# robotics-upo/social_force_window_planner

Hardware: AMD Instinct MI355X
Metric: scored trajectories/sec (v x w samples x steps) @ N pedestrians; cmd_vel match (higher is better)
Workload: dtype f64

## Files before the change

### social_force_window_planner_amd/csrc/sfw_kernels.hip

```cpp

#include "sfw_device.h"
#include "sfw_math.h"

#include <type_traits>

#include <math.h>
#include <stdlib.h>
#include <cmath>

namespace {

constexpr int WAVE = 64;

#pragma clang fp contract(off)

__device__ __forceinline__ unsigned cell_index(double a, double res, double inv_res) {
  const double q = a * inv_res;
  const double m = __builtin_trunc(q);
  const double d = q - m;
  if (d < 1e-9 || d > 1.0 - 1e-9) return static_cast<unsigned>(a / res);
  return static_cast<unsigned>(m);
}

__device__ __forceinline__ bool world_to_map(const sfw_launch &L, double inv_res, double wx, double wy, unsigned &mx,
// ... 563 lines not shown
template <bool BATCH> __device__ __forceinline__ late_launch late_args_of(late_launch rec) {
  if constexpr (!BATCH) {
    (void)rec;
    return late_args();
  } else {
    const __attribute__((address_space(4))) void *p = rec;
    asm volatile("" : "+s"(p));
    return static_cast<late_launch>(p);
  }
}

__device__ __forceinline__ void clock_probe(int which) {
  if (blockIdx.x != gridDim.x / 2 || threadIdx.x != 0) return;
  unsigned long long *const p = late_args()->clock_probe;
  if (!p) return;
  p[2 * which] = __builtin_readcyclecounter();
  p[2 * which + 1] = wall_clock64();
}

template <typename R> struct sfm_consts {
  sfwm::poly_consts pc;
  R lambda, neg_l2e_inv_gamma, l2_f_social, c_vel, c_ang;
};
struct agent_consts {
  double f_desired, inv_tau, dt, rr, inv_O, l2_f_obstacle, l2e_inv_sigma;
  double f_gaze, f_coherence, f_repulsion;
  const double *obstacles;
  int O, robot_id, obs_tasks;
};
__device__ __forceinline__ agent_consts load_agent_consts(late_launch La, bool f32) {
  agent_consts c;
  c.f_desired = La->k.f_desired;
  c.inv_tau = La->k.inv_tau;
  c.dt = La->dt;
  c.rr = La->k.rr;
  c.inv_O = La->k.inv_O;
  c.l2_f_obstacle = f32 ? static_cast<double>(La->k.f.l2_f_obstacle) : La->k.d.l2_f_obstacle;
  c.l2e_inv_sigma = f32 ? static_cast<double>(La->k.f.l2e_inv_sigma) : La->k.d.l2e_inv_sigma;
  c.f_gaze = La->p.sfm_force_factor_group_gaze;
  c.f_coherence = La->p.sfm_force_factor_group_coherence;
  c.f_repulsion = La->p.sfm_force_factor_group_repulsion;
  c.O = La->O;
  c.obstacles = La->obstacles;
  c.obs_tasks = La->k.obs_tasks;
  c.robot_id = La->agent_c[0].id;
  return c;
}

__device__ __forceinline__ double copysign_from(double mag, double sgn) { return __builtin_copysign(mag, sgn); }
__device__ __forceinline__ float copysign_from(float mag, double sgn) {
  return __builtin_copysignf(mag, static_cast<float>(sgn));
}

template <typename R, bool NORM_ONLY = false>
__device__ __forceinline__ void pair_force(const sfm_consts<R> &k, R dx, R dy, R wx, R wy, double cw, R &fx,
                                           R &fy) {
  using namespace sfwm;
  const R tiny = tiny_of<R>::v;
  R rd, dn, rl, il;
  const R d2 = fma(dx, dx, fma(dy, dy, tiny));
  rsqrt_sqrt(d2, rd, dn);
  const R ux = dx * rd, uy = dy * rd;
  const R ix = fma(k.lambda, wx, ux), iy = fma(k.lambda, wy, uy);
  const R l2 = fma(ix, ix, fma(iy, iy, tiny));
  rsqrt_sqrt(l2, rl, il);
  const R sn = fma(ix, uy, -(iy * ux));
  const R ncs = fma(-ix, ux, -(iy * uy));
  const R theta = angle_abs(k.pc, fabs(sn), ncs, rl, il);
  const R a = fmax(fma(dn * rl, k.neg_l2e_inv_gamma, k.l2_f_social), R(-1100));
  const R t2 = l2 * (theta * theta);
  R ev, ea;
#if SFW_SIGN_OF_ZERO
  exp2_fast2(k.pc, fma(k.c_vel, t2, a), fma(k.c_ang, t2, a), ev, ea);
#else
  exp2_fast2_gated(k.pc, fma(k.c_vel, t2, a), fma(k.c_ang, t2, a), cw, ev, ea);
#endif
  if constexpr (NORM_ONLY) {
    const R q = fma(ev, ev, ea * ea);
    R rq, nq;
    rsqrt_sqrt(fma(R(1), q, tiny), rq, nq);
    fx = q * rq;
    fy = R(0);
    return;
  }
  ea = copysign_from(ea, cw);
  const R gx = ix * rl, gy = iy * rl;
  fx = fma(ea, gy, -(ev * gx));
  fy = fma(-ev, gy, -(ea * gx));
}
template <typename R, bool NORM_ONLY = false>
__device__ __forceinline__ void pair_force_state(const sfm_consts<R> &k, double pix, double piy, double vix,
                                                 double viy, double pjx, double pjy, double vjx, double vjy,
                                                 R &fx, R &fy) {
  const double dx = pjx - pix, dy = pjy - piy, wx = vix - vjx, wy = viy - vjy;
  const double cw = fma(wx, dy, -(wy * dx));
  pair_force<R, NORM_ONLY>(k, R(dx), R(dy), R(wx), R(wy), cw, fx, fy);
}

__device__ __forceinline__ double fast_norm(double x, double y) {
  const double q = fma(x, x, y * y);
  double rs, sq;
  sfwm::rsqrt_sqrt(fmax(q, 1e-300), rs, sq);
  return q * rs;
}

__device__ __forceinline__ void desired_force(const agent_consts &k, double px, double py, double vx, double vy,
                                              bool has_goal, double gx, double gy, double gr, double dv, double &fx,
                                              double &fy) {
  const double ex = gx - px, ey = gy - py;
  double inv, en;
  sfwm::rsqrt_sqrt(fmax(fma(ex, ex, ey * ey), 1e-300), inv, en);
  if (has_goal && en > gr) {
    fx = k.f_desired * (ex * inv * dv - vx) * k.inv_tau;
    fy = k.f_desired * (ey * inv * dv - vy) * k.inv_tau;
  } else {
    fx = -vx * k.inv_tau;
    fy = -vy * k.inv_tau;
  }
}

constexpr int OBS_SEG = 16;
constexpr int OBS_AGENT_LANES = WAVE / OBS_SEG;
#ifndef SFW_OBS_KA
#define SFW_OBS_KA 4
#endif
constexpr int OBS_AGENTS_PER_LANE = SFW_OBS_KA;
typedef const __attribute__((address_space(4))) double *obs_global_ptr;
__device__ __forceinline__ obs_global_ptr obs_global(const double *obstacles) {
  return (obs_global_ptr)(const __attribute__((address_space(1))) double *)obstacles;
}
__device__ __forceinline__ double2 obs_point(const double2 *obs, int o) { return obs[o]; }
__device__ __forceinline__ double2 obs_point(obs_global_ptr obs, int o) { return double2{obs[2 * o], obs[2 * o + 1]}; }
#ifndef SFW_FLAT_PIPELINED
#define SFW_FLAT_PIPELINED false
#endif
#ifndef SFW_OBS_UNIFORM
#define SFW_OBS_UNIFORM 1
#endif
#ifndef SFW_OBS_UNIFORM_LDS
#define SFW_OBS_UNIFORM_LDS 1
#endif
#ifndef SFW_SKIP_EMPTY_K2
#define SFW_SKIP_EMPTY_K2 1
#endif
#ifndef SFW_OBS_UNROLL_SCALAR
#define SFW_OBS_UNROLL_SCALAR 4
#endif
template <typename R>
__device__ __forceinline__ void obstacle_term(const sfm_consts<R> &k, double2 q, double px, double py, R nis, R &ax, R &ay) {
// ... 162 lines not shown
    }
    if (seg_done) {
      tx += ax;
      ty += ay;
      ax = R(0);
      ay = R(0);
    }
  };
  auto advance = [&](int &o, int &e) {
    o += 4;
    if (o >= e) {
      o = e;
      e = min(e + L, O);
    }
    return o < O;
  };
  if (O > 0) {
    int o = 0, e = min(L, O);
    obs_group ga, gb;
    obs_group_issue(ga, obs);
    for (;;) {
      int o2 = o, e2 = e;
      const bool more = advance(o2, e2);
      obs_group_wait(ga);
      if (more) obs_group_issue(gb, obs + 2 * o2);
      eval(ga, min(4, e - o), o + 4 >= e);
      if (!more) break;
      o = o2;
      e = e2;
      const bool more2 = advance(o2, e2);
      obs_group_wait(gb);
      if (more2) obs_group_issue(ga, obs + 2 * o2);
      eval(gb, min(4, e - o), o + 4 >= e);
      if (!more2) break;
      o = o2;
      e = e2;
    }
  }
  tx_out = static_cast<double>(tx);
  ty_out = static_cast<double>(ty);
  scale = obstacle_scale<R>(k, c, radius);
}

__device__ __forceinline__ double swap_pair(double v) {
  const uint64_t u = __builtin_bit_cast(uint64_t, v);
  constexpr int QP_1032 = 0xB1;
  const uint32_t lo = static_cast<uint32_t>(__builtin_amdgcn_update_dpp(0, static_cast<int>(static_cast<uint32_t>(u)), QP_1032, 0xf, 0xf, true));
  const uint32_t hi = static_cast<uint32_t>(__builtin_amdgcn_update_dpp(0, static_cast<int>(static_cast<uint32_t>(u >> 32)), QP_1032, 0xf, 0xf, true));
  return __builtin_bit_cast(double, (static_cast<uint64_t>(hi) << 32) | lo);
}

struct lds_layout {
  double *px, *py, *vx, *vy, *fjx, *fjy, *fcx, *fcy;
  double2 *gcen;
  double2 *obs;
  sfw_robot_step *rsb;
  sfw_agent_const *ac;
  double *swp;
  double2 *opart;
  double *wr;
  double *oscale;
  int *hasgoal, *dead, *grp, *goff, *gmem;
  unsigned char *hasgoal8;
  int hg_stride;
  size_t bytes;
  static constexpr int REG_DEAD_CAP = 32;
  __host__ __device__ lds_layout(char *base, int A, int cap, int GA, int G, int O, int NG, int NM, bool consts,
                                 bool with_frc, bool obs_in_lds = false) {
    char *const base0 = base;
    auto take = [&](size_t n) {
      char *p = base;
      base += (n + 15) & ~size_t(15);
      return p;
    };
    const size_t plane = sizeof(double) * static_cast<size_t>(cap);
    px = reinterpret_cast<double *>(take(plane));
    py = reinterpret_cast<double *>(take(plane));
    vx = reinterpret_cast<double *>(take(plane));
    vy = reinterpret_cast<double *>(take(plane));
    fjx = reinterpret_cast<double *>(take(plane));
    fjy = reinterpret_cast<double *>(take(plane));
    if (with_frc) {
      fcx = reinterpret_cast<double *>(take(plane));
      fcy = reinterpret_cast<double *>(take(plane));
      rsb = reinterpret_cast<sfw_robot_step *>(take(sizeof(sfw_robot_step) * 2));
      swp = reinterpret_cast<double *>(take(sizeof(double) * GA));
      opart = reinterpret_cast<double2 *>(take(sizeof(double2) * (O > 0 ? (obs_in_lds ? 4 : 2) * 64 : 0)));
      wr = reinterpret_cast<double *>(take(sizeof(double) * (O > 0 ? 4 : 0)));
      oscale = reinterpret_cast<double *>(take(sizeof(double) * (O > 0 ? A : 0)));
      obs = reinterpret_cast<double2 *>(take(sizeof(double2) * (obs_in_lds ? O + 2 : 0)));
      if (!obs_in_lds) obs = nullptr;
      hasgoal8 = reinterpret_cast<unsigned char *>(take(static_cast<size_t>(GA)));
      hasgoal = nullptr;
      hg_stride = 1;
      dead = reinterpret_cast<int *>(take(sizeof(int) * G));
    } else {
      fcx = fcy = nullptr;
      opart = nullptr;
      wr = nullptr;
      oscale = nullptr;
      obs = nullptr;
      hasgoal = reinterpret_cast<int *>(take(plane));
      hasgoal8 = nullptr;
      hg_stride = 2;
      swp = reinterpret_cast<double *>(take(plane));
      dead = reinterpret_cast<int *>(take(sizeof(int) * REG_DEAD_CAP));
      rsb = reinterpret_cast<sfw_robot_step *>(take(sizeof(sfw_robot_step) * G));
    }
    ac = reinterpret_cast<sfw_agent_const *>(take(sizeof(sfw_agent_const) * (consts ? A : 0)));
    gcen = reinterpret_cast<double2 *>(take(sizeof(double2) * (NG > 0 ? G * NG : 0)));
    grp = reinterpret_cast<int *>(take(sizeof(int) * (NG > 0 ? A : 0)));
    goff = reinterpret_cast<int *>(take(sizeof(int) * (NG > 0 ? NG + 1 : 0)));
    gmem = reinterpret_cast<int *>(take(sizeof(int) * (NG > 0 && NM > 0 ? NM : 0)));
    bytes = static_cast<size_t>(base - base0);
  }
  __device__ __forceinline__ int hg(int sl) const { return hg_stride == 1 ? static_cast<int>(hasgoal8[sl]) : hasgoal[sl * hg_stride]; }
};
template <int CAP> struct reg_off {
  static constexpr int PY = 8 * CAP, VX = 16 * CAP, VY = 24 * CAP, FJX = 32 * CAP, FJY = 40 * CAP, HG = 48 * CAP, SW = 56 * CAP,
                       DEAD = 64 * CAP, RSB = 64 * CAP + 4 * lds_layout::REG_DEAD_CAP;
};

struct agent_k {
  double gx, gy, gr, dv, rad;
  int id;
};
__device__ __forceinline__ agent_k agent_k_of(const sfw_agent_const &c) {
  return agent_k{c.goal_x, c.goal_y, c.goal_radius, c.desired_velocity, c.radius, c.id};
}
__device__ __forceinline__ agent_k agent_k_lds(const lds_layout &s, int i) { return agent_k_of(s.ac[i]); }
__device__ __forceinline__ agent_k agent_k_global(const sfw_agent_const *agent_c, int i) { return agent_k_of(agent_c[i]); }

template <typename R>
__device__ double2 group_force(const sfm_consts<R> &k, const agent_consts &c, const lds_layout &s, int NG, int g, int A,
                               int i, int sl, double px, double py) {
  const sfw_agent_const ci = s.ac[i];
  const int q = s.grp[i];
  if (q < 0) return double2{0.0, 0.0};
  const int m0 = s.goff[q], m1 = s.goff[q + 1];
  if (m1 - m0 < 2) return double2{0.0, 0.0};
  const double n = static_cast<double>(m1 - m0), inv_n = sfwm::rcp_nr(n);
  const double2 csum = s.gcen[g * NG + q];
  const double cx = csum.x * inv_n, cy = csum.y * inv_n;
  const double ex = ci.goal_x - px, ey = ci.goal_y - py;
  double inv_en, en;
  sfwm::rsqrt_sqrt(fmax(fma(ex, ex, ey * ey), 1e-300), inv_en, en);
  const bool has_dir = s.hg(sl) && en > ci.goal_radius;
  const double ddx = has_dir ? ex * inv_en : 0.0, ddy = has_dir ? ey * inv_en : 0.0;
  double fx = 0.0, fy = 0.0;
  {
// ... 504 lines not shown
    if constexpr (GROUPS) add_group_forces(k, c);
      }

  const late_launch Le = late_args();
  if (Le->phase == SFW_PHASE_PREFIX) {
    sfw_cls_agent *const out_state = Le->out_state;
    const int64_t A_late = Le->A;
#pragma unroll
    for (int r = 0; r < NS; ++r)
      if (ok_[r] && static_cast<int>(g4_[r] >> 2) < Gn) {
        const uint32_t io = io_[r];
        sfw_cls_agent c;
        c.px = lds_at<double>(smem, io); c.py = lds_at<double>(smem, io + PY);
        c.vx = lds_at<double>(smem, io + VX); c.vy = lds_at<double>(smem, io + VY);
        c.fx = fx[r]; c.fy = fy[r]; c.sw = sw[r];
        const int2 cell = lds_at<int2>(smem, io + off::HG);
        c.hasgoal = cell.x;
        c.pad = 0;
        out_state[(first_local + static_cast<int64_t>(g4_[r] >> 2)) * A_late + (cell.y >> 1)] = c;
      }
    if (lane < Gn) Le->out_dead[first_local + lane] = s.dead[lane];
    clock_probe(1);
    return;
  }
  double sw_acc = 0.0;
#pragma unroll
  for (int r = 0; r < NS; ++r) {
    if (G == 1) sw_acc += ok_[r] ? sw[r] : 0.0;
    else if (ok_[r]) lds_at<double>(smem, io_[r] + off::SW) = sw[r];
  }
  finish_wave(s, lane, G, Gn, first_local, sw_acc);
  clock_probe(1);
}
template <typename R, int NS, bool GROUPS>
__global__ void __launch_bounds__(WAVE, (NS == 1 && !GROUPS) ? 6 : 1) sfw_social_kernel(const sfw_launch L, const int G) {
  sfwm::fp_mode_for_omod();
  extern __shared__ __attribute__((aligned(16))) char smem[];
  social_reg_wave<R, NS, GROUPS>(L, G, smem, blockIdx.x, gridDim.x);
}

__global__ void __launch_bounds__(256) sfw_pair_table_kernel(uint16_t *tab, int A, int n_entries, int n_dummy) {
  const int u = blockIdx.x * blockDim.x + threadIdx.x;
  if (u >= n_entries) return;
  const int P = A * (A - 1) / 2;
  int i = A + (u >= P ? (u - P) % n_dummy : 0), j = i;
  if (u < P) {
    const int row = u / A;
    i = u - row * A;
    j = i + row + 1;
    j = (j >= A) ? j - A : j;
  }
  tab[u] = static_cast<uint16_t>(8 * i);
  tab[n_entries + u] = static_cast<uint16_t>(8 * j);
}

__device__ __forceinline__ void load_pair_entries(const uint16_t *ti, const uint16_t *tj, uint32_t lane_off, uint32_t &io,
                                                  uint32_t &jo) {
#ifdef SFW_DBG_C_LOADS
  io = ti[lane_off / 2];
  jo = tj[lane_off / 2];
  return;
#endif
  asm volatile("s_nop 4\n\tglobal_load_ushort %0, %2, %3\n\tglobal_load_ushort %1, %2, %4"
               : "=&v"(io), "=&v"(jo)
               : "v"(lane_off), "s"(ti), "s"(tj));
}
__device__ __forceinline__ void wait_pair_entries(uint32_t &io, uint32_t &jo) {
  asm volatile("s_waitcnt vmcnt(0)" : "+v"(io), "+v"(jo));
}

#ifndef SFW_FIRST_PAIRS_IN_REGS
#define SFW_FIRST_PAIRS_IN_REGS 1
#endif
#ifndef SFW_FLAT_WAVES
#define SFW_FLAT_WAVES 5
#endif
#ifndef SFW_FLAT_WAVES_NOOBS
#define SFW_FLAT_WAVES_NOOBS 6
#endif
__device__ __forceinline__ void wave_sync() {
  __builtin_amdgcn_fence(__ATOMIC_RELEASE, "wavefront");
  __builtin_amdgcn_wave_barrier();
  __builtin_amdgcn_fence(__ATOMIC_ACQUIRE, "wavefront");
}
struct cycle_result {
  double social_work;
  int dead;
  int ready;
  int fdone;
  int legal;
  double base0, base;
};
__device__ __forceinline__ int cycle_wait_ready(const cycle_result *res, int need) {
  int r;
  while ((r = *const_cast<const volatile int *>(&res->ready)) < need) __builtin_amdgcn_s_sleep(1);
  __builtin_amdgcn_fence(__ATOMIC_ACQUIRE, "workgroup");
  return r;
}
#define K2_SYNC() do { if constexpr (CYCLE) wave_sync(); else __syncthreads(); } while (0)
template <typename R, bool GROUPS, int CAP, bool OBS, bool CYCLE, bool BATCH = false>
__device__ __forceinline__ void social_flat_wave(const sfw_launch &L, char *const smem, const k1s_lds *const k1, cycle_result *const res,
                                                 const unsigned bid, const unsigned nblk, const int64_t item_base,
                                                 const late_launch Lb = nullptr) {
  static_assert(CYCLE || !BATCH, "a batched wave is a cycle kernel's wave");
  const int lane = threadIdx.x;
  const int A = L.A, O = L.O;
  const int NG = GROUPS ? L.NG : 0;
  const int cap = CAP > 0 ? CAP : ((A + 2) & ~1);
  const int PY = 8 * cap, VX = 16 * cap, VY = 24 * cap, FJX = 32 * cap, FJY = 40 * cap, FCX = 48 * cap,
            FCY = 56 * cap;
  (void)FCX;
  (void)FCY;
  constexpr bool CONSTS_IN_LDS = GROUPS || CYCLE;
  const lds_layout s(smem, A, cap, A, 1, O, NG, GROUPS ? L.n_grp_mem : 0, CONSTS_IN_LDS, true, L.k.obs_lds != 0);
  const int64_t first_local = CYCLE ? static_cast<int64_t>(bid) : item_base + xcd_contiguous(bid, nblk, static_cast<unsigned>(L.n_xcd));
  const sfm_consts<R> k0 = make_consts<R, true>(L);
  const sfw_force_k<R> &fk = force_k<R>(L);
  const R s_lambda = sfwm::sgpr_const(fk.lambda), s_nig = sfwm::sgpr_const(fk.neg_l2e_inv_gamma), s_lfs = sfwm::sgpr_const(fk.l2_f_social),
          s_cvel = sfwm::sgpr_const(fk.c_vel), s_cang = sfwm::sgpr_const(fk.c_ang);
  constexpr bool F32 = sizeof(R) == 4;
  const int step_begin = L.step_begin, step_end = L.step_end;
  if constexpr (CYCLE) {
    stage_consts<GROUPS, CONSTS_IN_LDS>(L, s, lane);
    if (lane == 0) s.dead[0] = 0;
    wave_sync();
  } else {
    if (!stage_wave<GROUPS, GROUPS>(L, s, lane, 1, 1, first_local)) {
      if (L.phase == SFW_PHASE_SUFFIX) finish_wave(s, lane, 1, 1, first_local, 0.0);
      if (L.phase == SFW_PHASE_PREFIX && lane == 0) L.out_dead[first_local] = s.dead[0];
      return;
    }
  }
  if constexpr (!BATCH) clock_probe(0);
  const int64_t rsample_v = CYCLE ? 0 : robot_sample_of_item(L, first_local);
  const int64_t rsample = static_cast<int64_t>(
      (static_cast<uint64_t>(static_cast<uint32_t>(__builtin_amdgcn_readfirstlane(static_cast<int>(rsample_v >> 32)))) << 32) |
      static_cast<uint32_t>(__builtin_amdgcn_readfirstlane(static_cast<int>(rsample_v))));

  if (!CYCLE && L.resume) {
    const sfw_cls_agent *rec = L.in_state + source_class_of_item(L, first_local) * A;
    for (int sl = lane; sl < A; sl += WAVE) {
      const sfw_cls_agent c = rec[sl];
      s.px[sl] = c.px;
      s.py[sl] = c.py;
      s.vx[sl] = c.vx;
      s.vy[sl] = c.vy;
      s.hasgoal8[sl] = static_cast<unsigned char>(c.hasgoal != 0);
      s.swp[sl] = c.sw;
      s.fcx[sl] = c.fx;
      s.fcy[sl] = c.fy;
      s.fjx[sl] = s.fjy[sl] = 0.0;
    }
  } else {
    const agent_consts c0 = load_agent_consts(late_args_of<BATCH>(Lb), F32);
    for (int sl = lane; sl < A; sl += WAVE) {
      const double px = L.agent_pos[2 * sl], py = L.agent_pos[2 * sl + 1];
      const double vx = L.agent_vel[2 * sl], vy = L.agent_vel[2 * sl + 1];
      const sfw_agent_const c = L.agent_c[sl];
      s.px[sl] = px;
      s.py[sl] = py;
      s.vx[sl] = vx;
      s.vy[sl] = vy;
      s.hasgoal8[sl] = static_cast<unsigned char>(c.has_goal != 0);
      s.swp[sl] = 0.0;
      double fx = 0.0, fy = 0.0;
// ... 29 lines not shown
    K2_SYNC();
    for (int sl = lane; sl < A; sl += WAVE)
      if (s.grp[sl] >= 0) {
        atomicAdd(&s.gcen[s.grp[sl]].x, s.px[sl]);
        atomicAdd(&s.gcen[s.grp[sl]].y, s.py[sl]);
      }
    K2_SYNC();
    for (int sl = lane; sl < A; sl += WAVE)
      if (sl != 0) {
        const double2 gf = group_force<R>(k, c, s, NG, 0, A, sl, sl, s.px[sl], s.py[sl]);
        s.fcx[sl] += gf.x;
        s.fcy[sl] += gf.y;
      }
    K2_SYNC();
  };
  if constexpr (GROUPS) {
    if (!L.resume) add_group_forces(k0, load_agent_consts(late_args_of<BATCH>(Lb), F32));
  }

  const int P = A * (A - 1) / 2;
  const int n_it = (P + WAVE - 1) / WAVE;
  const uint16_t *const tab_i = L.pair_tab, *const tab_j = L.pair_tab + static_cast<size_t>(n_it) * WAVE;
  const uint32_t lane_off = 2u * static_cast<uint32_t>(lane);

  const int64_t unit_vel_v = CYCLE ? 0 : L.rstep_stride + vel_row_of(L, rsample);
  const int64_t unit_pos = rsample,
                unit_vel = static_cast<int64_t>(
                    (static_cast<uint64_t>(static_cast<uint32_t>(__builtin_amdgcn_readfirstlane(static_cast<int>(unit_vel_v >> 32)))) << 32) |
                    static_cast<uint32_t>(__builtin_amdgcn_readfirstlane(static_cast<int>(unit_vel_v))));
  auto fetch_robot = [&](const sfw_unit *ptab, int64_t row_units, int st, int buf) {
    if constexpr (CYCLE) return;
    int l2 = lane;
    asm volatile("" : "+v"(l2));
    if (l2 < 2) {
      const char *src = reinterpret_cast<const char *>(ptab + static_cast<int64_t>(st) * row_units + (l2 ? unit_vel : unit_pos));
      __builtin_amdgcn_global_load_lds((const __attribute__((address_space(1))) void *)src,
                                       (__attribute__((address_space(3))) void *)(reinterpret_cast<char *>(s.rsb + buf)), 16,
                                       0, 0);
    }
  };
  if (step_begin < step_end) fetch_robot(L.ptab, L.row_units, step_begin, step_begin & 1);
  constexpr bool FIRST_IN_REGS = SFW_FIRST_PAIRS_IN_REGS && CAP == 64;
  uint32_t i0 = 0, j0 = 0;
  if constexpr (FIRST_IN_REGS) {
    if (n_it > 0) {
      load_pair_entries(tab_i, tab_j, lane_off, i0, j0);
      wait_pair_entries(i0, j0);
    }
  }

#if defined(SFW_ABL_HALF_LDS)
  double abl_ix = s.px[lane < A ? lane : 0], abl_iy = s.py[lane < A ? lane : 0], abl_fx = 0.0, abl_fy = 0.0;
#endif
  auto pair_at = [&](const sfm_consts<R> &k, uint32_t io, uint32_t jo) {
    R qx, qy;
    if constexpr (CAP > 0) {
      double pix, piy, vix, viy, pjx, pjy, vjx, vjy;
#if defined(SFW_ABL_NOREAD)
      pix = static_cast<double>(io); piy = 1.0; vix = 0.3; viy = 0.5; pjx = static_cast<double>(jo) * 0.37; pjy = -3.0; vjx = 0.25; vjy = static_cast<double>(jo) * 0.001;
#elif defined(SFW_ABL_HALF_LDS)
      pix = abl_ix; piy = abl_iy; vix = 0.3; viy = 0.5;
      asm volatile("ds_read_b64 %0, %4\n\tds_read_b64 %1, %4 offset:%5\n\tds_read_b64 %2, %4 offset:%6\n\tds_read_b64 %3, %4 offset:%7\n\ts_waitcnt lgkmcnt(0)"
                   : "=&v"(pjx), "=&v"(pjy), "=&v"(vjx), "=&v"(vjy) : "v"(jo), "n"(8 * CAP), "n"(16 * CAP), "n"(24 * CAP) : "memory");
#else
      lds_pair_state<8 * CAP, 16 * CAP, 24 * CAP>(io, jo, pix, piy, vix, viy, pjx, pjy, vjx, vjy);
#endif
#if defined(SFW_ABL_NOMATH)
      qx = R(pix + pjy - vjx); qy = R(piy - pjx + vix * viy + vjy);
#else
      pair_force_state<R>(k, pix, piy, vix, viy, pjx, pjy, vjx, vjy, qx, qy);
#endif
    } else {
      pair_force_state<R>(k, lds_at<double>(smem, io), lds_at<double>(smem, io + PY), lds_at<double>(smem, io + VX),
                          lds_at<double>(smem, io + VY), lds_at<double>(smem, jo), lds_at<double>(smem, jo + PY),
                          lds_at<double>(smem, jo + VX), lds_at<double>(smem, jo + VY), qx, qy);
    }
#if defined(SFW_ABL_NOATOM)
    asm volatile("" :: "v"(qx), "v"(qy));
#elif defined(SFW_ABL_HALF_LDS)
    abl_fx += static_cast<double>(qx);
    abl_fy += static_cast<double>(qy);
    atomicAdd(&lds_at<double>(smem, jo + FJX), static_cast<double>(qx));
    atomicAdd(&lds_at<double>(smem, jo + FJY), static_cast<double>(qy));
#else
    atomicAdd(&lds_at<double>(smem, io + FCX), static_cast<double>(qx));
    atomicAdd(&lds_at<double>(smem, io + FCY), static_cast<double>(qy));
    atomicAdd(&lds_at<double>(smem, jo + FJX), static_cast<double>(qx));
    atomicAdd(&lds_at<double>(smem, jo + FJY), static_cast<double>(qy));
#endif
  };

  [[maybe_unused]] int cyc_ready = 0;
  for (int step = step_begin; step < step_end; ++step) {
    sfm_consts<R> k = k0;
    if constexpr (OBS) {
      k.pc.leading_here();
      k.lambda = sfwm::vgpr_copy_here(s_lambda);
      k.neg_l2e_inv_gamma = sfwm::vgpr_copy_here(s_nig);
      k.l2_f_social = sfwm::vgpr_copy_here(s_lfs);
      k.c_vel = sfwm::vgpr_copy_here(s_cvel);
      k.c_ang = sfwm::vgpr_copy_here(s_cang);
    }
    if constexpr (FIRST_IN_REGS) {
    if (n_it > 0) {
      uint32_t ia, ja, ib, jb;
      const uint16_t *ti = tab_i + WAVE, *tj = tab_j + WAVE;
      int left = n_it - 1;
      if (left >= 1) load_pair_entries(ti, tj, lane_off, ia, ja);
      pair_at(k, i0, j0);
      ti += WAVE;
      tj += WAVE;
      for (; left >= 2; left -= 2, ti += 2 * WAVE, tj += 2 * WAVE) {
        wait_pair_entries(ia, ja);
        load_pair_entries(ti, tj, lane_off, ib, jb);
        pair_at(k, ia, ja);
        wait_pair_entries(ib, jb);
        if (left > 2) load_pair_entries(ti + WAVE, tj + WAVE, lane_off, ia, ja);
        pair_at(k, ib, jb);
      }
      if (left == 1) {
        wait_pair_entries(ia, ja);
        pair_at(k, ia, ja);
      }
    }
    asm volatile("s_waitcnt vmcnt(0)" ::: "memory");
    } else {
    if (n_it > 0) {
      uint32_t ia, ja, ib, jb;
      load_pair_entries(tab_i, tab_j, lane_off, ia, ja);
      int left = n_it;
      const uint16_t *ti = tab_i + WAVE, *tj = tab_j + WAVE;
      for (; left >= 2; left -= 2, ti += 2 * WAVE, tj += 2 * WAVE) {
        wait_pair_entries(ia, ja);
        load_pair_entries(ti, tj, lane_off, ib, jb);
        pair_at(k, ia, ja);
        wait_pair_entries(ib, jb);
        if (left > 2) load_pair_entries(ti + WAVE, tj + WAVE, lane_off, ia, ja);
        pair_at(k, ib, jb);
      }
      if (left == 1) {
        wait_pair_entries(ia, ja);
        pair_at(k, ia, ja);
      }
    } else {
      asm volatile("s_waitcnt vmcnt(0)" ::: "memory");
    }
    }
    K2_SYNC();
#if defined(SFW_ABL_HALF_LDS)
    if (lane < A) { s.fcx[lane] += abl_fx; s.fcy[lane] += abl_fy; abl_ix = s.px[lane] + 1e-3; abl_iy = s.py[lane]; abl_fx = abl_fy = 0.0; }
#endif
    const late_launch La = late_args_of<BATCH>(Lb);
    const agent_consts c = load_agent_consts(La, F32);
    const sfw_agent_const *const agent_c = La->agent_c;
    if constexpr (CYCLE) {
      if (step >= cyc_ready) cyc_ready = cycle_wait_ready(res, step + 1);
    }
    const sfw_robot_step rs = CYCLE ? sfw_robot_step{k1->xs[step + 1], k1->ys[step + 1], k1->vxs[step], k1->vys[step]} : s.rsb[step & 1];
    if (step + 1 < step_end) fetch_robot(La->ptab, La->row_units, step + 1, (step + 1) & 1);
    const bool with_obs = OBS && c.O > 0;
    int lane_s = lane;
    asm volatile("" : "+v"(lane_s));
#if defined(SFW_ABL_NOAGENT)
    for (int sl = lane_s; sl < 0; sl += WAVE) {
#else
    for (int sl = lane_s; sl < A; sl += WAVE) {
#endif
      const agent_k ak = CONSTS_IN_LDS ? agent_k_lds(s, sl) : agent_k_global(agent_c, sl);
      double px = s.px[sl], py = s.py[sl], vx = s.vx[sl], vy = s.vy[sl];
      double nfx, nfy;
      int hg = s.hasgoal8[sl];
      const int hg0 = hg;
      bool contact;
      const double w = agent_step<R>(k, c, rs, ak, sl == 0, ak.id != c.robot_id, hg, contact, px, py, vx, vy,
                                     s.fcx[sl] - s.fjx[sl], s.fcy[sl] - s.fjy[sl], nfx, nfy);
      if (sl != 0 && hg0) s.hasgoal8[sl] = static_cast<unsigned char>(hg);
#if !defined(SFW_ABL_NOATOM) && !defined(SFW_ABL_NOREAD) && !defined(SFW_ABL_NOMATH) && !defined(SFW_ABL_KEEPALIVE) && !defined(SFW_ABL_HALF_LDS)
      if (contact) s.dead[0] = 2 + step;
#endif
      if (sl == 0 && with_obs) {
        s.wr[0] = w;
      } else {
        s.swp[sl] += w;
      }
      if (sl == 0) {
        px = rs.x;
        py = rs.y;
        vx = rs.vx;
        vy = rs.vy;
      }
      if (!(sl == 0 && with_obs)) {
        s.px[sl] = px;
        s.py[sl] = py;
        s.vx[sl] = vx;
        s.vy[sl] = vy;
      }
      s.fcx[sl] = nfx;
      s.fcy[sl] = nfy;
      s.fjx[sl] = 0.0;
      s.fjy[sl] = 0.0;
    }
    if (with_obs) {
      K2_SYNC();
      if (c.obs_tasks) {
        const int Lseg = (c.O + OBS_SEG - 1) / OBS_SEG, seg = lane >> 2, sub = lane & (OBS_AGENT_LANES - 1);
        const int ob = min(seg * Lseg, c.O), oe = min(ob + Lseg, c.O);
        const R nis = sfwm::vgpr_const(static_cast<R>(-c.l2e_inv_sigma));
        const double2 *const pts_g = reinterpret_cast<const double2 *>(c.obstacles);
        const obs_lds_ptr pts_l = (obs_lds_ptr)s.obs;
        const bool in_lds = s.obs != nullptr;
        const double *const part = reinterpret_cast<const double *>(s.opart);
        constexpr int KA = OBS_AGENTS_PER_LANE;
        for (int a0 = 0; a0 < A; a0 += OBS_AGENT_LANES * KA) {
          const int nj = min(KA, (A - a0 + OBS_AGENT_LANES - 1) / OBS_AGENT_LANES);
          double pxj[KA], pyj[KA];
          R axj[KA + 1], ayj[KA + 1];
#pragma unroll
          for (int j = 0; j < KA; ++j) {
            pxj[j] = pyj[j] = 0.0;
            if (j < nj) {
              const int a = min(a0 + sub + OBS_AGENT_LANES * j, A - 1);
              pxj[j] = s.px[a];
              pyj[j] = s.py[a];
            }
          }
#pragma unroll
          for (int j = 0; j <= KA; ++j) axj[j] = ayj[j] = R(0);
          auto run = [&](auto pts) {
// ... 47 lines not shown
                  R t = R(0);
#pragma unroll
                  for (int q = 0; q < OBS_SEG; ++q) t += static_cast<R>(v[q]);
                  const double f = static_cast<double>(t) * sc;
                  const double f_other = swap_pair(f);
                  if (a != 0) *acc = fma(static_cast<double>(t), sc, acc0);
                  else if (comp == 0) s.swp[0] += wr0 + fast_norm(f, f_other);
                }
                K2_SYNC();
              }
            }
          };
          if (in_lds && nj > 2) reduce(std::integral_constant<int, (KA >= 4 ? 4 : 2)>{});
          else reduce(std::integral_constant<int, 2>{});
        }
      } else {
        for (int a = lane; a < A; a += WAVE) {
          const double rad = CONSTS_IN_LDS ? s.ac[a].radius : agent_c[a].radius;
          double tx, ty, sc;
          obstacle_sums<R, SFW_FLAT_PIPELINED>(k, c, obs_global(c.obstacles), s.px[a], s.py[a], rad, tx, ty, sc);
          if (a == 0) {
            s.swp[0] += s.wr[0] + fast_norm(tx * sc, ty * sc);
          } else {
            s.fcx[a] = fma(tx, sc, s.fcx[a]);
            s.fcy[a] = fma(ty, sc, s.fcy[a]);
          }
        }
        K2_SYNC();
      }
      if (lane == 0) {
        s.px[0] = rs.x;
        s.py[0] = rs.y;
        s.vx[0] = rs.vx;
        s.vy[0] = rs.vy;
      }
    }
    if (const double *const pin = La->pin_rest) {
      if (pin_at_rest(pin, rs))
        for (int sl = lane_s; sl < A; sl += WAVE) {
          if (sl == 0) {
            s.fcx[0] += pin[2];
            s.fcy[0] += pin[3];
          } else {
            s.swp[sl] += pin[4 + sl];
          }
        }
    }
    K2_SYNC();
    if (s.dead[0] != 0) break;
    if constexpr (GROUPS) add_group_forces(k, c);
  }
  asm volatile("s_waitcnt vmcnt(0)" ::: "memory");
  const late_launch Le = late_args_of<BATCH>(Lb);
  if (Le->phase == SFW_PHASE_PREFIX) {
    sfw_cls_agent *rec = Le->out_state + first_local * A;
    for (int sl = lane; sl < A; sl += WAVE) {
      sfw_cls_agent c;
      c.px = s.px[sl]; c.py = s.py[sl]; c.vx = s.vx[sl]; c.vy = s.vy[sl];
      c.fx = s.fcx[sl]; c.fy = s.fcy[sl]; c.sw = s.swp[sl];
      c.hasgoal = s.hasgoal8[sl];
      c.pad = 0;
      rec[sl] = c;
    }
    if (lane == 0) Le->out_dead[first_local] = s.dead[0];
    if constexpr (!BATCH) clock_probe(1);
    return;
  }
  double sw_acc = 0.0;
  for (int sl = lane; sl < A; sl += WAVE) sw_acc += s.swp[sl];
  if constexpr (CYCLE) {
    for (int off = WAVE / 2; off > 0; off >>= 1) sw_acc += __shfl_down(sw_acc, off, WAVE);
    if (lane == 0) {
      res->social_work = sw_acc;
      res->dead = s.dead[0];
    }
  } else {
    finish_wave(s, lane, 1, 1, first_local, sw_acc);
  }
  if constexpr (!BATCH) clock_probe(1);
}
#undef K2_SYNC
template <typename R, bool GROUPS, int CAP, bool OBS>
__global__ void __launch_bounds__(WAVE, (GROUPS || CAP == 0) ? 1 : OBS ? SFW_FLAT_WAVES : SFW_FLAT_WAVES_NOOBS) sfw_social_kernel_flat(const sfw_launch L, const int G_unused) {
  sfwm::fp_mode_for_omod();
  extern __shared__ __attribute__((aligned(16))) char smem[];
  (void)G_unused;
  social_flat_wave<R, GROUPS, CAP, OBS, false>(L, smem, nullptr, nullptr, blockIdx.x, gridDim.x, L.item_base);
}
template <typename R>
__global__ void __launch_bounds__(WAVE, 6) sfw_social_kernel_mixed(const sfw_launch L, const int G, const int n_reg, const int keep) {
  sfwm::fp_mode_for_omod();
  extern __shared__ __attribute__((aligned(16))) char smem[];
  if (blockIdx.x < static_cast<unsigned>(n_reg)) {
    sfw_launch Lr = L;
    if (Lr.phase == SFW_PHASE_PREFIX) Lr.n_cls = keep;
    else Lr.chunk_count = keep;
    social_reg_wave<R, 1, false>(Lr, G, smem, blockIdx.x, static_cast<unsigned>(n_reg));
  } else {
    social_flat_wave<R, false, 64, false, false>(L, smem, nullptr, nullptr, blockIdx.x - static_cast<unsigned>(n_reg),
                                                 gridDim.x - static_cast<unsigned>(n_reg), keep);
  }
}

__device__ __forceinline__ bool sel_less(const sfw_sel &a, const sfw_sel &b) {
  if (a.cost != b.cost) return a.cost < b.cost;
  if (a.neg_linvel != b.neg_linvel) return a.neg_linvel < b.neg_linvel;
// ... 375 lines not shown
  const double l2e = 1.4426950408889634074;
  d.neg_l2e_inv_gamma = -l2e / p.sfm_gamma;
  d.l2_f_social = std::log2(p.sfm_force_factor_social);
  d.c_vel = -(p.sfm_n_prime * p.sfm_n_prime) * (p.sfm_gamma * p.sfm_gamma) * l2e;
  d.c_ang = -(p.sfm_n * p.sfm_n) * (p.sfm_gamma * p.sfm_gamma) * l2e;
  d.l2_f_obstacle = p.sfm_force_factor_obstacle > 0 ? std::log2(p.sfm_force_factor_obstacle) : -1000.0;
  d.l2e_inv_sigma = l2e / p.sfm_force_sigma_obstacle;
  sfw_force_k<float> &f = L.k.f;
  f.lambda = static_cast<float>(d.lambda);
  f.neg_l2e_inv_gamma = static_cast<float>(d.neg_l2e_inv_gamma);
  f.l2_f_social = static_cast<float>(d.l2_f_social);
  f.c_vel = static_cast<float>(d.c_vel);
  f.c_ang = static_cast<float>(d.c_ang);
  f.l2_f_obstacle = static_cast<float>(d.l2_f_obstacle);
  f.l2e_inv_sigma = static_cast<float>(d.l2e_inv_sigma);
  L.k.f_desired = p.sfm_force_factor_desired;
  L.k.inv_tau = 1.0 / p.sfm_relaxation_time;
  L.k.rr = static_cast<double>(static_cast<float>(p.robot_radius) * static_cast<float>(p.robot_radius));
  L.k.inv_O = L.O > 0 ? 1.0 / L.O : 0.0;
  {
    const int A = L.A, O = L.O, Lseg = (O + OBS_SEG - 1) / OBS_SEG;
    const int full = A / (OBS_AGENT_LANES * OBS_AGENTS_PER_LANE), rest = (A % (OBS_AGENT_LANES * OBS_AGENTS_PER_LANE) + OBS_AGENT_LANES - 1) / OBS_AGENT_LANES;
    const double red = 40.0;
    const double c_tasks = full * (27.0 * Lseg * OBS_AGENTS_PER_LANE + 2 * red) + (rest ? 27.0 * Lseg * rest + ((rest + 1) / 2) * red : 0.0);
    const double c_lane = 27.0 * O * ((A + WAVE - 1) / WAVE);
    L.k.obs_tasks = (O > 0 && c_tasks < c_lane) ? 1 : 0;
  }
}

static int flat_cap(int A) { return A < 64 ? 64 : A < 104 ? 104 : A < 128 ? 128 : A < 208 ? 208 : A < 256 ? 256 : 0; }
static int flat_cap_runtime(int A) { return (A + 2) & ~1; }

static size_t lds_bytes_for(const wave_plan &pl, int A, int O, int NG, int n_grp_mem, bool obs_lds);
static bool obs_in_lds(const wave_plan &pl, int A, int O, int NG, int n_grp_mem, int64_t items, int cus) {
  return pl.flat && O > 0 && items <= static_cast<int64_t>(8) * cus && lds_bytes_for(pl, A, O, NG, n_grp_mem, true) <= 64 * 1024;
}
static size_t lds_bytes_for(const wave_plan &pl, int A, int O, int NG, int n_grp_mem, bool obs_lds) {
  if (pl.flat) {
    const int c = flat_cap(A);
    return lds_layout(nullptr, A, c > 0 ? c : flat_cap_runtime(A), A, 1, O, NG, n_grp_mem, NG > 0, true, obs_lds).bytes;
  }
  (void)obs_lds;
  return lds_layout(nullptr, A, WAVE * pl.ns, pl.G * A, pl.G, O, NG, n_grp_mem, true, false).bytes;
}

size_t sfw_social_lds_bytes(int A, int O, int NG, int n_grp_mem, int64_t T, int form, int cus) {
  const wave_plan pl = plan_for(A, T, O, form, cus);
  const size_t a = lds_bytes_for(pl, A, O, NG, n_grp_mem, obs_in_lds(pl, A, O, NG, n_grp_mem, T, cus));
  const wave_plan fl{1, 0, true};
  const size_t b = (A >= 2 || O > 0) ? lds_bytes_for(fl, A, O, NG, n_grp_mem, obs_in_lds(fl, A, O, NG, n_grp_mem, 1, cus)) : 0;
  return a > b ? a : b;
}

int64_t sfw_pair_table_entries(int A) {
  const int64_t P = static_cast<int64_t>(A) * (A - 1) / 2;
  const int64_t n = (P + WAVE - 1) / WAVE * WAVE;
  return 2 * (n > 0 ? n : WAVE);
}

hipError_t sfw_launch_pair_table(uint16_t *tab, int A, hipStream_t stream) {
  const int n = static_cast<int>(sfw_pair_table_entries(A) / 2);
  const int cap = flat_cap(A) > 0 ? flat_cap(A) : flat_cap_runtime(A);
  hipLaunchKernelGGL(sfw_pair_table_kernel, dim3((n + 255) / 256), dim3(256), 0, stream, tab, A, n, cap - A);
  return hipGetLastError();
}

static bool sfw_k1a_threads() {
  const char *e = std::getenv("SFW_K1A_THREADS");
  return e && e[0] == '1';
}

bool sfw_rollout_is_fused(const sfw_launch &L) { return L.chunk_count <= 2048 && L.S <= K1_SMALL_MAX_STEPS; }

hipError_t sfw_launch_rollout_poses(const sfw_launch &L, hipStream_t stream) {
  if (L.chunk_count <= 0) return hipSuccess;
  if (sfw_rollout_is_fused(L)) {
    hipLaunchKernelGGL(sfw_rollout_small_kernel, dim3(static_cast<unsigned>(L.chunk_count)), dim3(K1_SMALL_BLOCK), 0, stream, L);
    return hipGetLastError();
  }
  const int block = 64;
  if (sfw_k1a_threads()) {
    const unsigned grid = static_cast<unsigned>((L.chunk_count + block - 1) / block);
    hipLaunchKernelGGL(sfw_rollout_kernel, dim3(grid), dim3(block), 0, stream, L);
    return hipGetLastError();
  }
  constexpr int per_wave = WAVE / K1A_TEAM;
  const unsigned grid = static_cast<unsigned>((L.chunk_count + per_wave - 1) / per_wave);
  hipLaunchKernelGGL(sfw_rollout_team_kernel, dim3(grid), dim3(block), 0, stream, L);
  return hipGetLastError();
}

hipError_t sfw_launch_rollout_costmap(const sfw_launch &L, hipStream_t stream) {
  if (L.chunk_count <= 0 || sfw_rollout_is_fused(L)) return hipSuccess;
  {
    const int block = 256;
    const int64_t n = L.chunk_count * L.S;
    const unsigned grid = static_cast<unsigned>((n + block - 1) / block);
    hipLaunchKernelGGL(sfw_footprint_kernel, dim3(grid), dim3(block), 0, stream, L);
  }
  {
    const int block = 256;
    const unsigned grid = static_cast<unsigned>((L.chunk_count + block - 1) / block);
    hipLaunchKernelGGL(sfw_costmap_scan_kernel, dim3(grid), dim3(block), 0, stream, L);
  }
  return hipGetLastError();
}

hipError_t sfw_launch_rollout(const sfw_launch &L, hipStream_t stream) {
  hipError_t e = sfw_launch_rollout_poses(L, stream);
  return e != hipSuccess ? e : sfw_launch_rollout_costmap(L, stream);
}

template <typename K> static hipError_t launch_social_as(K kernel, const sfw_launch &L, int G, unsigned grid,
                                                          size_t lds, hipStream_t stream) {
// ... 284 lines not shown
```

Baseline: 7.599 million.

## Reuse robot-pedestrian pair exponentials from pair pass for social work score

During the all-pairs social force pass, pairs involving the robot now export their exponential terms (ev, ea) and write them into new LDS planes. The writes use exec-masked ds_write with per-iteration robot masks that the pair-table kernel precomputes. The agent step then rebuilds the robot's social-work norm from these cached values instead of calling a second pair_force evaluation per pedestrian. A final extra pass computes the missing last-step contribution. This removes one duplicated transcendental evaluation per pedestrian per step. In exchange it adds LDS footprint, scalar mask loads, inline asm exec manipulation, and a changed pair-table size.

New measurement: 7.585 million (median of 2 runs). Within noise of the previous version (-0.2%).

```diff
diff --git a/social_force_window_planner_amd/csrc/sfw_kernels.hip b/social_force_window_planner_amd/csrc/sfw_kernels.hip
--- a/social_force_window_planner_amd/csrc/sfw_kernels.hip
+++ b/social_force_window_planner_amd/csrc/sfw_kernels.hip
@@ -639,9 +639,16 @@
   return __builtin_copysignf(mag, static_cast<float>(sgn));
 }
 
-template <typename R, bool NORM_ONLY = false>
-__device__ __forceinline__ void pair_force(const sfm_consts<R> &k, R dx, R dy, R wx, R wy, double cw, R &fx,
-                                           R &fy) {
+template <typename R> __device__ __forceinline__ R pair_norm(R ev, R ea) {
+  const R q = fma(ev, ev, ea * ea);
+  R rq, nq;
+  sfwm::rsqrt_sqrt(fma(R(1), q, tiny_of<R>::v), rq, nq);
+  return q * rq;
+}
+
+template <typename R, bool NORM_ONLY = false, bool EXPORT = false>
+__device__ __forceinline__ void pair_force_ex(const sfm_consts<R> &k, R dx, R dy, R wx, R wy, double cw, R &fx,
+                                              R &fy, R &ev_out, R &ea_out) {
   using namespace sfwm;
   const R tiny = tiny_of<R>::v;
   R rd, dn, rl, il;
@@ -663,17 +670,28 @@
   exp2_fast2_gated(k.pc, fma(k.c_vel, t2, a), fma(k.c_ang, t2, a), cw, ev, ea);
 #endif
   if constexpr (NORM_ONLY) {
-    const R q = fma(ev, ev, ea * ea);
-    R rq, nq;
-    rsqrt_sqrt(fma(R(1), q, tiny), rq, nq);
-    fx = q * rq;
+    if constexpr (EXPORT) {
+      ev_out = ev;
+      ea_out = ea;
+    }
+    fx = pair_norm<R>(ev, ea);
     fy = R(0);
     return;
   }
   ea = copysign_from(ea, cw);
+  if constexpr (EXPORT) {
+    ev_out = ev;
+    ea_out = ea;
+  }
   const R gx = ix * rl, gy = iy * rl;
   fx = fma(ea, gy, -(ev * gx));
   fy = fma(-ev, gy, -(ea * gx));
+}
+template <typename R, bool NORM_ONLY = false>
+__device__ __forceinline__ void pair_force(const sfm_consts<R> &k, R dx, R dy, R wx, R wy, double cw, R &fx,
+                                           R &fy) {
+  R ev_unused, ea_unused;
+  pair_force_ex<R, NORM_ONLY, false>(k, dx, dy, wx, wy, cw, fx, fy, ev_unused, ea_unused);
 }
 template <typename R, bool NORM_ONLY = false>
 __device__ __forceinline__ void pair_force_state(const sfm_consts<R> &k, double pix, double piy, double vix,
@@ -682,6 +700,14 @@
   const double dx = pjx - pix, dy = pjy - piy, wx = vix - vjx, wy = viy - vjy;
   const double cw = fma(wx, dy, -(wy * dx));
   pair_force<R, NORM_ONLY>(k, R(dx), R(dy), R(wx), R(wy), cw, fx, fy);
+}
+template <typename R>
+__device__ __forceinline__ void pair_force_state_export(const sfm_consts<R> &k, double pix, double piy, double vix,
+                                                        double viy, double pjx, double pjy, double vjx, double vjy,
+                                                        R &fx, R &fy, R &ev, R &ea) {
+  const double dx = pjx - pix, dy = pjy - piy, wx = vix - vjx, wy = viy - vjy;
+  const double cw = fma(wx, dy, -(wy * dx));
+  pair_force_ex<R, false, true>(k, R(dx), R(dy), R(wx), R(wy), cw, fx, fy, ev, ea);
 }
 
 __device__ __forceinline__ double fast_norm(double x, double y) {
@@ -950,6 +976,7 @@
 
 struct lds_layout {
   double *px, *py, *vx, *vy, *fjx, *fjy, *fcx, *fcy;
+  double *wev, *wea;
   double2 *gcen;
   double2 *obs;
   sfw_robot_step *rsb;
@@ -963,6 +990,8 @@
   int hg_stride;
   size_t bytes;
   static constexpr int REG_DEAD_CAP = 32;
+  static constexpr int HANDOVER_CAP_MAX = 128;
+  __host__ __device__ static constexpr bool has_handover(int cap) { return cap <= HANDOVER_CAP_MAX; }
   __host__ __device__ lds_layout(char *base, int A, int cap, int GA, int G, int O, int NG, int NM, bool consts,
                                  bool with_frc, bool obs_in_lds = false) {
     char *const base0 = base;
@@ -981,6 +1010,8 @@
     if (with_frc) {
       fcx = reinterpret_cast<double *>(take(plane));
       fcy = reinterpret_cast<double *>(take(plane));
+      wev = reinterpret_cast<double *>(take(has_handover(cap) ? plane : 0));
+      wea = reinterpret_cast<double *>(take(has_handover(cap) ? plane : 0));
       rsb = reinterpret_cast<sfw_robot_step *>(take(sizeof(sfw_robot_step) * 2));
       swp = reinterpret_cast<double *>(take(sizeof(double) * GA));
       opart = reinterpret_cast<double2 *>(take(sizeof(double2) * (O > 0 ? (obs_in_lds ? 4 : 2) * 64 : 0)));
@@ -994,6 +1025,7 @@
       dead = reinterpret_cast<int *>(take(sizeof(int) * G));
     } else {
       fcx = fcy = nullptr;
+      wev = wea = nullptr;
       opart = nullptr;
       wr = nullptr;
       oscale = nullptr;
@@ -1604,6 +1636,12 @@
   }
   tab[u] = static_cast<uint16_t>(8 * i);
   tab[n_entries + u] = static_cast<uint16_t>(8 * j);
+  const unsigned long long robot_i = __ballot(u < P && i == 0), robot_j = __ballot(u < P && j == 0);
+  if (threadIdx.x % WAVE == 0) {
+    unsigned long long *const masks = reinterpret_cast<unsigned long long *>(tab + 2 * static_cast<size_t>(n_entries));
+    masks[2 * (u / WAVE)] = robot_i;
+    masks[2 * (u / WAVE) + 1] = robot_j;
+  }
 }
 
 __device__ __forceinline__ void load_pair_entries(const uint16_t *ti, const uint16_t *tj, uint32_t lane_off, uint32_t &io,
@@ -1619,6 +1657,46 @@
 }
 __device__ __forceinline__ void wait_pair_entries(uint32_t &io, uint32_t &jo) {
   asm volatile("s_waitcnt vmcnt(0)" : "+v"(io), "+v"(jo));
+}
+
+struct pair_masks { uint64_t robot_i, robot_j; };
+typedef const __attribute__((address_space(4))) uint64_t *pair_mask_ptr;
+__device__ __forceinline__ pair_mask_ptr pair_mask_table(const uint16_t *behind_the_arrays) {
+  return reinterpret_cast<pair_mask_ptr>(reinterpret_cast<uintptr_t>(behind_the_arrays));
+}
+__device__ __forceinline__ pair_masks load_pair_masks(pair_mask_ptr m) { return pair_masks{m[0], m[1]}; }
+
+template <int WEV, int WEA> __device__ __forceinline__ void hand_over(uint32_t io, uint32_t jo, double ev, double ea, const pair_masks &m) {
+  asm volatile(
+      "s_mov_b64 vcc, exec\n\t"
+      "s_mov_b64 exec, %4\n\t"
+      "ds_write_b64 %1, %2 offset:%6\n\t"
+      "ds_write_b64 %1, %3 offset:%7\n\t"
+      "s_mov_b64 exec, %5\n\t"
+      "ds_write_b64 %0, %2 offset:%6\n\t"
+      "ds_write_b64 %0, %3 offset:%7\n\t"
+      "s_mov_b64 exec, vcc"
+      :
+      : "v"(io), "v"(jo), "v"(ev), "v"(ea), "s"(m.robot_i), "s"(m.robot_j), "n"(WEV), "n"(WEA)
+      : "vcc", "memory");
+}
+template <int WEV, int WEA> __device__ __forceinline__ void hand_over(uint32_t io, uint32_t jo, float ev, float ea, const pair_masks &m) {
+  asm volatile(
+      "s_mov_b64 vcc, exec\n\t"
+      "s_mov_b64 exec, %4\n\t"
+      "ds_write_b32 %1, %2 offset:%6\n\t"
+      "ds_write_b32 %1, %3 offset:%7\n\t"
+      "s_mov_b64 exec, %5\n\t"
+      "ds_write_b32 %0, %2 offset:%6\n\t"
+      "ds_write_b32 %0, %3 offset:%7\n\t"
+      "s_mov_b64 exec, vcc"
+      :
+      : "v"(io), "v"(jo), "v"(ev), "v"(ea), "s"(m.robot_i), "s"(m.robot_j), "n"(WEV), "n"(WEA)
+      : "vcc", "memory");
+}
+template <typename R> __device__ __forceinline__ R handed_over(const double *cell) {
+  if constexpr (sizeof(R) == 4) return *reinterpret_cast<const float *>(cell);
+  else return *cell;
 }
 
 #ifndef SFW_FIRST_PAIRS_IN_REGS
@@ -1663,6 +1741,9 @@
             FCY = 56 * cap;
   (void)FCX;
   (void)FCY;
+  constexpr bool HANDOVER = CAP > 0 && lds_layout::has_handover(CAP);
+  constexpr int WEV = 64 * CAP, WEA = 72 * CAP;
+  const bool handover = HANDOVER && L.pin_rest == nullptr;
   constexpr bool CONSTS_IN_LDS = GROUPS || CYCLE;
   const lds_layout s(smem, A, cap, A, 1, O, NG, GROUPS ? L.n_grp_mem : 0, CONSTS_IN_LDS, true, L.k.obs_lds != 0);
   const int64_t first_local = CYCLE ? static_cast<int64_t>(bid) : item_base + xcd_contiguous(bid, nblk, static_cast<unsigned>(L.n_xcd));
@@ -1798,7 +1879,9 @@
 #if defined(SFW_ABL_HALF_LDS)
   double abl_ix = s.px[lane < A ? lane : 0], abl_iy = s.py[lane < A ? lane : 0], abl_fx = 0.0, abl_fy = 0.0;
 #endif
-  auto pair_at = [&](const sfm_consts<R> &k, uint32_t io, uint32_t jo) {
+  auto pair_at = [&](const sfm_consts<R> &k, uint32_t io, uint32_t jo, auto ho, const pair_masks &m) {
+    constexpr bool HO = decltype(ho)::value;
+    (void)m;
     R qx, qy;
     if constexpr (CAP > 0) {
       double pix, piy, vix, viy, pjx, pjy, vjx, vjy;
@@ -1814,7 +1897,13 @@
 #if defined(SFW_ABL_NOMATH)
       qx = R(pix + pjy - vjx); qy = R(piy - pjx + vix * viy + vjy);
 #else
-      pair_force_state<R>(k, pix, piy, vix, viy, pjx, pjy, vjx, vjy, qx, qy);
+      if constexpr (HO) {
+        R ev, ea;
+        pair_force_state_export<R>(k, pix, piy, vix, viy, pjx, pjy, vjx, vjy, qx, qy, ev, ea);
+        hand_over<WEV, WEA>(io, jo, ev, ea, m);
+      } else {
+        pair_force_state<R>(k, pix, piy, vix, viy, pjx, pjy, vjx, vjy, qx, qy);
+      }
 #endif
     } else {
       pair_force_state<R>(k, lds_at<double>(smem, io), lds_at<double>(smem, io + PY), lds_at<double>(smem, io + VX),
@@ -1847,26 +1936,40 @@
       k.c_vel = sfwm::vgpr_copy_here(s_cvel);
       k.c_ang = sfwm::vgpr_copy_here(s_cang);
     }
+    auto pair_pass = [&](auto ho) {
+    constexpr bool HO = decltype(ho)::value;
+    [[maybe_unused]] const pair_mask_ptr mk = pair_mask_table(tab_j + static_cast<size_t>(n_it) * WAVE);
+    [[maybe_unused]] pair_masks ma{0, 0}, mb{0, 0};
     if constexpr (FIRST_IN_REGS) {
     if (n_it > 0) {
       uint32_t ia, ja, ib, jb;
       const uint16_t *ti = tab_i + WAVE, *tj = tab_j + WAVE;
       int left = n_it - 1;
-      if (left >= 1) load_pair_entries(ti, tj, lane_off, ia, ja);
-      pair_at(k, i0, j0);
+      int it = 1;
+      pair_masks m0{0, 0};
+      if constexpr (HO) m0 = load_pair_masks(mk);
+      if (left >= 1) {
+        load_pair_entries(ti, tj, lane_off, ia, ja);
+        if constexpr (HO) ma = load_pair_masks(mk + 2);
+      }
+      pair_at(k, i0, j0, ho, m0);
       ti += WAVE;
       tj += WAVE;
-      for (; left >= 2; left -= 2, ti += 2 * WAVE, tj += 2 * WAVE) {
+      for (; left >= 2; left -= 2, ti += 2 * WAVE, tj += 2 * WAVE, it += 2) {
         wait_pair_entries(ia, ja);
         load_pair_entries(ti, tj, lane_off, ib, jb);
-        pair_at(k, ia, ja);
+        if constexpr (HO) mb = load_pair_masks(mk + 2 * (it + 1));
+        pair_at(k, ia, ja, ho, ma);
         wait_pair_entries(ib, jb);
-        if (left > 2) load_pair_entries(ti + WAVE, tj + WAVE, lane_off, ia, ja);
-        pair_at(k, ib, jb);
+        if (left > 2) {
+          load_pair_entries(ti + WAVE, tj + WAVE, lane_off, ia, ja);
+          if constexpr (HO) ma = load_pair_masks(mk + 2 * (it + 2));
+        }
+        pair_at(k, ib, jb, ho, mb);
       }
       if (left == 1) {
         wait_pair_entries(ia, ja);
-        pair_at(k, ia, ja);
+        pair_at(k, ia, ja, ho, ma);
       }
     }
     asm volatile("s_waitcnt vmcnt(0)" ::: "memory");
@@ -1874,23 +1977,36 @@
     if (n_it > 0) {
       uint32_t ia, ja, ib, jb;
       load_pair_entries(tab_i, tab_j, lane_off, ia, ja);
+      if constexpr (HO) ma = load_pair_masks(mk);
       int left = n_it;
+      int it = 0;
       const uint16_t *ti = tab_i + WAVE, *tj = tab_j + WAVE;
-      for (; left >= 2; left -= 2, ti += 2 * WAVE, tj += 2 * WAVE) {
+      for (; left >= 2; left -= 2, ti += 2 * WAVE, tj += 2 * WAVE, it += 2) {
         wait_pair_entries(ia, ja);
         load_pair_entries(ti, tj, lane_off, ib, jb);
-        pair_at(k, ia, ja);
+        if constexpr (HO) mb = load_pair_masks(mk + 2 * (it + 1));
+        pair_at(k, ia, ja, ho, ma);
         wait_pair_entries(ib, jb);
-        if (left > 2) load_pair_entries(ti + WAVE, tj + WAVE, lane_off, ia, ja);
-        pair_at(k, ib, jb);
+        if (left > 2) {
+          load_pair_entries(ti + WAVE, tj + WAVE, lane_off, ia, ja);
+          if constexpr (HO) ma = load_pair_masks(mk + 2 * (it + 2));
+        }
+        pair_at(k, ib, jb, ho, mb);
       }
       if (left == 1) {
         wait_pair_entries(ia, ja);
-        pair_at(k, ia, ja);
+        pair_at(k, ia, ja, ho, ma);
       }
     } else {
       asm volatile("s_waitcnt vmcnt(0)" ::: "memory");
     }
+    }
+    };
+    if constexpr (HANDOVER) {
+      if (handover) pair_pass(std::true_type{});
+      else pair_pass(std::false_type{});
+    } else {
+      pair_pass(std::false_type{});
     }
     K2_SYNC();
 #if defined(SFW_ABL_HALF_LDS)
@@ -1918,8 +2034,13 @@
       int hg = s.hasgoal8[sl];
       const int hg0 = hg;
       bool contact;
-      const double w = agent_step<R>(k, c, rs, ak, sl == 0, ak.id != c.robot_id, hg, contact, px, py, vx, vy,
-                                     s.fcx[sl] - s.fjx[sl], s.fcy[sl] - s.fjy[sl], nfx, nfy);
+      const bool wp_on = ak.id != c.robot_id;
+      double w = agent_step<R>(k, c, rs, ak, sl == 0, wp_on && !handover, hg, contact, px, py, vx, vy,
+                               s.fcx[sl] - s.fjx[sl], s.fcy[sl] - s.fjy[sl], nfx, nfy);
+      if constexpr (HANDOVER) {
+        if (handover && sl != 0 && wp_on && step != step_begin)
+          w = static_cast<double>(pair_norm<R>(handed_over<R>(s.wev + sl), handed_over<R>(s.wea + sl)));
+      }
       if (sl != 0 && hg0) s.hasgoal8[sl] = static_cast<unsigned char>(hg);
 #if !defined(SFW_ABL_NOATOM) && !defined(SFW_ABL_NOREAD) && !defined(SFW_ABL_NOMATH) && !defined(SFW_ABL_KEEPALIVE) && !defined(SFW_ABL_HALF_LDS)
       if (contact) s.dead[0] = 2 + step;
@@ -2073,6 +2194,30 @@
   }
   asm volatile("s_waitcnt vmcnt(0)" ::: "memory");
   const late_launch Le = late_args_of<BATCH>(Lb);
+  if constexpr (HANDOVER) {
+    if (handover && step_begin < step_end && s.dead[0] == 0) {
+      sfm_consts<R> k = k0;
+      if constexpr (OBS) {
+        k.pc.leading_here();
+        k.lambda = sfwm::vgpr_copy_here(s_lambda);
+        k.neg_l2e_inv_gamma = sfwm::vgpr_copy_here(s_nig);
+        k.l2_f_social = sfwm::vgpr_copy_here(s_lfs);
+        k.c_vel = sfwm::vgpr_copy_here(s_cvel);
+        k.c_ang = sfwm::vgpr_copy_here(s_cang);
+      }
+      const sfw_agent_const *const agent_c = Le->agent_c;
+      const int robot_id = agent_c[0].id;
+      const double rx = s.px[0], ry = s.py[0], rvx = s.vx[0], rvy = s.vy[0];
+      for (int sl = lane; sl < A; sl += WAVE) {
+        const int id = CONSTS_IN_LDS ? s.ac[sl].id : agent_c[sl].id;
+        if (sl != 0 && id != robot_id) {
+          R qn, unused;
+          pair_force_state<R, true>(k, s.px[sl], s.py[sl], s.vx[sl], s.vy[sl], rx, ry, rvx, rvy, qn, unused);
+          s.swp[sl] += static_cast<double>(qn);
+        }
+      }
+    }
+  }
   if (Le->phase == SFW_PHASE_PREFIX) {
     sfw_cls_agent *rec = Le->out_state + first_local * A;
     for (int sl = lane; sl < A; sl += WAVE) {
@@ -2554,14 +2699,18 @@
   return a > b ? a : b;
 }
 
-int64_t sfw_pair_table_entries(int A) {
+static int64_t pair_table_array_entries(int A) {
   const int64_t P = static_cast<int64_t>(A) * (A - 1) / 2;
   const int64_t n = (P + WAVE - 1) / WAVE * WAVE;
-  return 2 * (n > 0 ? n : WAVE);
+  return n > 0 ? n : WAVE;
+}
+int64_t sfw_pair_table_entries(int A) {
+  const int64_t n = pair_table_array_entries(A);
+  return 2 * n + n / WAVE * 2 * static_cast<int64_t>(sizeof(uint64_t) / sizeof(uint16_t));
 }
 
 hipError_t sfw_launch_pair_table(uint16_t *tab, int A, hipStream_t stream) {
-  const int n = static_cast<int>(sfw_pair_table_entries(A) / 2);
+  const int n = static_cast<int>(pair_table_array_entries(A));
   const int cap = flat_cap(A) > 0 ? flat_cap(A) : flat_cap_runtime(A);
   hipLaunchKernelGGL(sfw_pair_table_kernel, dim3((n + 255) / 256), dim3(256), 0, stream, tab, A, n, cap - A);
   return hipGetLastError();
```
